# xinyiW915/ReLaX-VQA

Measured on AMD Instinct MI355X. Metric: clips/sec (32 sampled frames, 1080p) feature extraction, higher is better.
Workload: dtype f32 (fp32-grade split-operand arithmetic, fp32 accumulate: the whole ViT (GEMMs and attention), ResNet-50's stem, layer3 / layer4, and in layer1 / layer2 the 3x3 convolutions, every conv3 (back to back with its 3x3), the downsample convolutions and layer2's conv1 on fp32 operands as 2 fp16 planes x

## Files before the change

relax-vqa_amd/csrc/gemm_h2.hip:

```cpp
#include "relax_internal.h"
#include "host_logic.h"
#include "h2.h"
#include "gelu.h"

#ifndef H3_EP_FETCH_AHEAD
#define H3_EP_FETCH_AHEAD 0
#endif
#ifndef H2_STAMP
#define H2_STAMP(i_)
#define H2_STAMPS_BEFORE_LAUNCH(h_, p_, units_)
#define H2_STAMPS_AFTER_LAUNCH(h_, p_, units_, s_)
#endif
#ifndef H3_ABL_NO_A
#define H3_ABL_NO_A(taps_, perimg_, p_) false
#define H3_ABL_NO_OUT_H2(taps_, p_) false
#endif
#ifndef H3_KSTEP
#define H3_KSTEP(k_) (k_)
#endif

namespace relax {

typedef float h2k_f32x4 __attribute__((ext_vector_type(4)));
typedef float f32x4 __attribute__((ext_vector_type(4)));
// ... 90 lines not shown
    hipLaunchKernelGGL(to_h2_rows_kernel, dim3((unsigned)((rows + 3) / 4)), dim3(256), 0, s, x, ld, static_cast<char*>(y), K, rows, inv_scale);
    RELAX_HIP_CHECK(h, hipGetLastError());
    return RELAX_OK;
}

struct H2Params {
    const char* a;
    const char* w;
    const float* colscale;
    const float* rowscale;
    const float* bias;
    const float* residual;
    float* out;
    char* out_h2;
    float out_scale;
    float* partial;
    int M, N, K;
    int act;
    int no_split;
    int tiles_m, tiles_n, ntiles, group_m;
    int full_tiles, nsplit;
    int pixels, H, W, Cin, Ho, Wo, KW, stride, pad;
    int rows_per_img;
    const float* img_in_inv;
    const float* img_out_scale;
    unsigned* amax_out;
    const char* residual_h2;
    const float* img_res_inv;
    float* gap;
    int out_rows, gap_rows;
    unsigned long long* stamps;
};

__device__ inline int xcd_remap_h2(int b, int nwg) {
    const int q = nwg >> 3, r = nwg & 7, xcd = b & 7;
    const int base = xcd < r ? xcd * (q + 1) : r * (q + 1) + (xcd - r) * q;
    return base + (b >> 3);
}

#define H2_DMA(rsrc_, lds_off_, voff_, soff_)                                                                             \
    __builtin_amdgcn_raw_ptr_buffer_load_lds(rsrc_, (__attribute__((address_space(3))) void*)(smem + (lds_off_)), 16,     \
                                             voff_, soff_, 0, 0)
[[maybe_unused]] constexpr unsigned kH2OutOfRange = 0x80000000u;
constexpr int64_t kH2MaxRecords = 0x7ffffff0;

constexpr int H2_BM = 256, H2_BN = 256;
constexpr int H2_STAGE = (H2_BM + H2_BN) * kH2ChunkBytes;
constexpr int H2_PIECES = H2_STAGE / 1024;
[[maybe_unused]] constexpr int H2_PPW = H2_PIECES / 8;

template <int NSTG>
__global__ __launch_bounds__(512, 2) void gemm_h2(const H2Params p) {
#if __HIP_DEVICE_COMPILE__
    constexpr int BM = H2_BM, BN = H2_BN, STAGE = H2_STAGE, PPW = H2_PPW;
    extern __shared__ __attribute__((aligned(16))) char smem[];
    const int tid = threadIdx.x;
    const int lane = tid & 63;
    const int wave = __builtin_amdgcn_readfirstlane(tid >> 6);
    const int wm = wave >> 2, wn = wave & 3;

    int tile, kt_begin, kt_end, slice = -1, split_tile = 0;
    {
        const int nk_all = p.K >> 4;
        const int b = blockIdx.x;
        if (b < p.full_tiles) {
            tile = xcd_remap_h2(b, p.full_tiles);
            kt_begin = 0;
            kt_end = nk_all;
        } else {
            const int u = b - p.full_tiles;
            split_tile = u / p.nsplit;
            slice = u - split_tile * p.nsplit;
            tile = p.full_tiles + split_tile;
            kt_begin = (int)((int64_t)nk_all * slice / p.nsplit);
            kt_end = (int)((int64_t)nk_all * (slice + 1) / p.nsplit);
        }
    }
    int tm, tn;
    {
        const int per_group = p.group_m * p.tiles_n;
        const int g = tile / per_group;
        const int first = g * p.group_m;
        const int gsz = p.tiles_m - first < p.group_m ? p.tiles_m - first : p.group_m;
        const int w = tile - g * per_group;
        tm = first + w % gsz;
        tn = w / gsz;
    }
    const int m0 = tm * BM;
    const int n0 = tn * BN;
    H2_STAMP(0);

    const int64_t row_bytes = (int64_t)p.K * 4;
    __amdgpu_buffer_rsrc_t rsrc_a, rsrc_w;
    {
        const int64_t left = (int64_t)(p.M - m0) * row_bytes;
        rsrc_a = __builtin_amdgcn_make_buffer_rsrc(const_cast<char*>(p.a + (int64_t)m0 * row_bytes), 0,
                                                   (int)(left < kH2MaxRecords ? left : kH2MaxRecords), 0x00020000);
        rsrc_w = __builtin_amdgcn_make_buffer_rsrc(const_cast<char*>(p.w + (int64_t)n0 * row_bytes), 0, (int)(BN * row_bytes), 0x00020000);
    }
    unsigned voff_a, voff_w;
    {
        const int r = 32 * wave + (lane >> 1);
        voff_a = m0 + r < p.M ? (unsigned)(r * (int)row_bytes + (lane & 1) * 16) : kH2OutOfRange;
        voff_w = (unsigned)(r * (int)row_bytes + (lane & 1) * 16);
    }
    int d_kt = kt_begin;
#define H2_ISSUE_PIECE(st_, j_)                                                                                         \
    {                                                                                                                   \
        const int soff_ = d_kt * kH2ChunkBytes + ((j_) >> 1) * 32;                                                      \
        const int dst_ = (st_) * STAGE + ((j_) >> 1) * (STAGE / 2) + ((j_) & 1) * (BM * 32) + wave * 1024;               \
        if (((j_) & 1) == 0) { H2_DMA(rsrc_a, dst_, voff_a, soff_); }                                                    \
        else { H2_DMA(rsrc_w, dst_, voff_w, soff_); }                                                                    \
    }
#define H2_ISSUE(st_)                                                                                                   \
    {                                                                                                                   \
        _Pragma("unroll") for (int j = 0; j < PPW; ++j) H2_ISSUE_PIECE(st_, j);                                         \
        ++d_kt;                                                                                                         \
    }

    floatx4 acc[8][4];
#pragma unroll
    for (int i = 0; i < 8; ++i)
#pragma unroll
        for (int j = 0; j < 4; ++j)
#pragma unroll
            for (int r = 0; r < 4; ++r) acc[i][j][r] = 0.f;

    const int r16 = lane & 15, g16 = lane >> 4;
    const int a_hl = (g16 >> 1) * (STAGE / 2) + (wm * 128 + r16) * 32 + ((g16 & 1) << 4);
    const int b_hh = (BM + wn * 64 + r16) * 32 + ((g16 & 1) << 4);
    h2k_f16x8 xb[2][4][2], ya[2];
#define H2_READ_XB(set_, sp_)                                                                                           \
    _Pragma("unroll") for (int y = 0; y < 4; ++y) {                                                                     \
        xb[set_][y][0] = *reinterpret_cast<const h2k_f16x8*>((sp_) + b_hh + y * 16 * 32);                               \
        xb[set_][y][1] = *reinterpret_cast<const h2k_f16x8*>((sp_) + b_hh + y * 16 * 32 + STAGE / 2);                   \
    }
#define H2_READ_A(buf_, e_, sp_)                                                                                        \
    {                                                                                                                   \
        ya[buf_] = *reinterpret_cast<const h2k_f16x8*>((sp_) + a_hl + (e_) * 16 * 32);                                  \
        __builtin_amdgcn_sched_barrier(0);                        \
    }
#define H2_MFMAS(set_, buf_, e_)                                                                                        \
    {                                                                                                                   \
        _Pragma("unroll") for (int y = 0; y < 4; ++y)                                                                   \
            acc[e_][y] = __builtin_amdgcn_mfma_f32_16x16x32_f16(ya[buf_], xb[set_][y][1], acc[e_][y], 0, 0, 0);         \
        _Pragma("unroll") for (int y = 0; y < 4; ++y)                                                                   \
            acc[e_][y] = __builtin_amdgcn_mfma_f32_16x16x32_f16(ya[buf_], xb[set_][y][0], acc[e_][y], 0, 0, 0);         \
        __builtin_amdgcn_sched_barrier(0);        \
    }
#define H2_REGION(xs_, st_, has_next_, has_d_)                                                                          \
    {                                                                                                                   \
        const char* sn_ = smem + (((st_) + 1) % NSTG) * STAGE;                                                          \
        if (has_next_) {                                                                                                \
            if (has_d_) asm volatile("s_waitcnt vmcnt(%0) lgkmcnt(0)" ::"n"((NSTG - 2) * PPW) : "memory");              \
            else asm volatile("s_waitcnt vmcnt(0) lgkmcnt(0)" ::: "memory");                                            \
            __builtin_amdgcn_s_barrier();                                                                               \
            H2_READ_XB((xs_) ^ 1, sn_);                                                                                 \
            H2_READ_A(0, 0, sn_);                                                                                       \
        }                                                                                                               \
        H2_MFMAS(xs_, 1, 7);                                                                                            \
        if (has_next_) {                                                                                                \
            _Pragma("unroll") for (int e = 0; e < 7; ++e) {                                                             \
                H2_READ_A((e + 1) & 1, e + 1, sn_);                                                                     \
                if ((has_d_) && e < PPW) H2_ISSUE_PIECE(st_, e);                                                        \
                H2_MFMAS((xs_) ^ 1, e & 1, e);                                                                          \
            }                                                                                                           \
            if (has_d_) ++d_kt;                                                                                         \
        }                                                                                                               \
    }

    const int nk = kt_end - kt_begin;
    {
        const int pre = nk < NSTG ? nk : NSTG;
        for (int i = 0; i < pre; ++i) H2_ISSUE(i);
        if (pre >= 4) asm volatile("s_waitcnt vmcnt(%0)" ::"n"(3 * PPW) : "memory");
        else if (pre == 3) asm volatile("s_waitcnt vmcnt(%0)" ::"n"(2 * PPW) : "memory");
        else if (pre == 2) asm volatile("s_waitcnt vmcnt(%0)" ::"n"(PPW) : "memory");
        else asm volatile("s_waitcnt vmcnt(0)" ::: "memory");
    }
    __builtin_amdgcn_s_barrier();
    H2_READ_XB(0, smem);
    H2_READ_A(0, 0, smem);
    H2_STAMP(1);
#pragma unroll
    for (int e = 0; e < 7; ++e) {
        H2_READ_A((e + 1) & 1, e + 1, smem);
        H2_MFMAS(0, e & 1, e);
    }
    {
        constexpr int PERIOD = (NSTG % 2 == 0) ? NSTG : 2 * NSTG;
        int k = 0;
        for (; k + PERIOD + NSTG <= nk; k += PERIOD) {
#pragma unroll
            for (int i = 0; i < PERIOD; ++i) H2_REGION(i & 1, i % NSTG, true, true);
        }
        for (; k < nk; k += PERIOD) {
#pragma unroll
            for (int i = 0; i < PERIOD; ++i)
                if (k + i < nk) H2_REGION(i & 1, i % NSTG, k + i + 1 < nk, k + i + NSTG < nk);
        }
    }
#undef H2_REGION
#undef H2_MFMAS
#undef H2_READ_A
#undef H2_READ_XB
#undef H2_ISSUE
#undef H2_ISSUE_PIECE
    H2_STAMP(2);
    __syncthreads();

    float* stg = reinterpret_cast<float*>(smem);
    constexpr int LDC = BN + 4;
    constexpr int EP_ROWS = 64;
    constexpr int C8 = BN / 8;
    constexpr int NT = 512;
    static_assert(EP_ROWS * LDC * 4 <= NSTG * STAGE, "epilogue pass must fit the staging LDS");
    constexpr int EP_STEP = NT / C8;
    constexpr int EP_ITERS = EP_ROWS / EP_STEP;
    const bool planes = p.out_h2 != nullptr;
    const int lcA = planes ? (tid % C8) * 8 : (tid % C8) * 4;
    const int lcB = planes ? lcA + 4 : lcA + BN / 2;
    const int lr0 = tid / C8;
    const f32x4 zero4 = {0.f, 0.f, 0.f, 0.f};
    f32x4 bias_a = zero4, bias_b = zero4, cs_a = zero4, cs_b = zero4;
    if (slice < 0) {
        cs_a = *reinterpret_cast<const f32x4*>(p.colscale + n0 + lcA);
        cs_b = *reinterpret_cast<const f32x4*>(p.colscale + n0 + lcB);
        if (p.bias) {
            bias_a = *reinterpret_cast<const f32x4*>(p.bias + n0 + lcA);
            bias_b = *reinterpret_cast<const f32x4*>(p.bias + n0 + lcB);
        }
    }
    const bool interior = m0 + BM <= p.M;
#pragma unroll
    for (int pass = 0; pass < BM / EP_ROWS; ++pass) {
        if (pass > 0) __syncthreads();
        f32x4 ra[EP_ITERS], rb[EP_ITERS];
        float rs[EP_ITERS];
#pragma unroll
        for (int it = 0; it < EP_ITERS; ++it) {
            const int m = m0 + pass * EP_ROWS + it * EP_STEP + lr0;
            ra[it] = zero4;
            rb[it] = zero4;
            rs[it] = 1.f;
            if (slice < 0 && (interior || m < p.M)) {
                if (p.residual) {
                    const float* r = p.residual + (int64_t)m * p.N + n0;
                    ra[it] = *reinterpret_cast<const f32x4*>(r + lcA);
                    rb[it] = *reinterpret_cast<const f32x4*>(r + lcB);
                }
                if (p.rowscale) rs[it] = p.rowscale[m];
            }
        }
#pragma unroll
        for (int x = 0; x < 8; ++x) {
            const int rb0 = wm * 128 + x * 16;
            if (rb0 / EP_ROWS == pass) {
#pragma unroll
                for (int y = 0; y < 4; ++y)
#pragma unroll
                    for (int r = 0; r < 4; ++r) stg[(rb0 % EP_ROWS + 4 * g16 + r) * LDC + wn * 64 + y * 16 + r16] = acc[x][y][r];
            }
        }
        __syncthreads();
#pragma unroll
        for (int it = 0; it < EP_ITERS; ++it) {
            const int lr = it * EP_STEP + lr0;
            const int trow = pass * EP_ROWS + lr;
            const int m = m0 + trow;
            if (!interior && m >= p.M) continue;
            f32x4 va = *reinterpret_cast<const f32x4*>(stg + lr * LDC + lcA);
            f32x4 vb = *reinterpret_cast<const f32x4*>(stg + lr * LDC + lcB);
            if (slice >= 0) {
                float* o = p.partial + ((int64_t)split_tile * p.nsplit + slice) * (BM * BN) + (int64_t)trow * BN;
                *reinterpret_cast<f32x4*>(o + lcA) = va;
                *reinterpret_cast<f32x4*>(o + lcB) = vb;
                continue;
            }
            va = va * (cs_a * rs[it]) + bias_a;
            vb = vb * (cs_b * rs[it]) + bias_b;
            if (p.residual) {
                va += ra[it];
                vb += rb[it];
            }
            if (p.act == 1) {
                va = (f32x4){fmaxf(va.x, 0.f), fmaxf(va.y, 0.f), fmaxf(va.z, 0.f), fmaxf(va.w, 0.f)};
                vb = (f32x4){fmaxf(vb.x, 0.f), fmaxf(vb.y, 0.f), fmaxf(vb.z, 0.f), fmaxf(vb.w, 0.f)};
            } else if (p.act == 2) {
                va = gelu_erf4(va);
                vb = gelu_erf4(vb);
            }
            const int64_t o = (int64_t)m * p.N + n0;
            if (p.out) {
                *reinterpret_cast<f32x4*>(p.out + o + lcA) = va;
                *reinterpret_cast<f32x4*>(p.out + o + lcB) = vb;
            }
            if (p.out_h2) store_h2_x8(p.out_h2 + (int64_t)m * ((int64_t)p.N * 4), n0 + lcA, va, vb, p.out_scale);
        }
    }
    H2_STAMP(3);
#endif
}

constexpr int H3_STAGE = (H2_BM + H2_BN) * 128;
constexpr int H3_NSTG = 2;

__device__ inline float dpp_row_max(float v) {
#define H3_DPP_MAX(CTRL_) v = fmaxf(v, __builtin_bit_cast(float, __builtin_amdgcn_update_dpp(0, __builtin_bit_cast(int, v), CTRL_, 0xf, 0xf, true)))
    H3_DPP_MAX(0xB1);
    H3_DPP_MAX(0x4E);
    H3_DPP_MAX(0x141);
    H3_DPP_MAX(0x140);
#undef H3_DPP_MAX
    return v;
}

template <bool FOUR, bool TAPS = false, bool PERIMG = false>
__global__ __launch_bounds__(512, 2) void gemm_h3(const H2Params p) {
#if __HIP_DEVICE_COMPILE__
    constexpr int BM = H2_BM, BN = H2_BN, STAGE = H3_STAGE, NSTG = H3_NSTG, IMG = STAGE / 2;
    extern __shared__ __attribute__((aligned(16))) char smem[];
    const int tid = threadIdx.x;
    const int lane = tid & 63;
    const int wave = __builtin_amdgcn_readfirstlane(tid >> 6);
    const int wm = wave >> 2, wn = wave & 3;

    int tile, kt_begin, kt_end, slice = -1, split_tile = 0;
    {
        const int nk_all = p.K >> 5;
        const int b = blockIdx.x;
        if (b < p.full_tiles) {
            tile = xcd_remap_h2(b, p.full_tiles);
            kt_begin = 0;
            kt_end = nk_all;
        } else {
            const int u = b - p.full_tiles;
            split_tile = u / p.nsplit;
            slice = u - split_tile * p.nsplit;
            tile = p.full_tiles + split_tile;
            kt_begin = (int)((int64_t)nk_all * slice / p.nsplit);
            kt_end = (int)((int64_t)nk_all * (slice + 1) / p.nsplit);
        }
    }
    int tm, tn;
    {
        const int per_group = p.group_m * p.tiles_n;
        const int g = tile / per_group;
        const int first = g * p.group_m;
        const int gsz = p.tiles_m - first < p.group_m ? p.tiles_m - first : p.group_m;
        const int w = tile - g * per_group;
        tm = first + w % gsz;
        tn = w / gsz;
    }
    const int m0 = tm * BM;
    const int n0 = tn * BN;
#ifdef H3_STAGGER
    if (PERIMG && !TAPS && blockIdx.x < 256 && (blockIdx.x & 3)) {
        const unsigned long long t0 = __builtin_amdgcn_s_memtime(), wait = (unsigned long long)(blockIdx.x & 3) * (H3_STAGGER);
        while (__builtin_amdgcn_s_memtime() - t0 < wait) __builtin_amdgcn_s_sleep(32);
    }
#endif
    H2_STAMP(0);

    const int64_t row_bytes = (int64_t)p.K * 4;
    const int64_t arow_bytes = p.pixels ? (int64_t)p.Cin * 4 : row_bytes;
    const int img0 = p.pixels ? m0 / (p.Ho * p.Wo) : 0;
    __amdgpu_buffer_rsrc_t rsrc_a, rsrc_w;
    {
        const int64_t base = p.pixels ? (int64_t)img0 * p.H * p.W * arow_bytes : (int64_t)m0 * arow_bytes;
        const int64_t total = p.pixels ? (int64_t)(p.M / (p.Ho * p.Wo)) * p.H * p.W * arow_bytes : (int64_t)p.M * arow_bytes;
        const int64_t left = total - base;
        rsrc_a = __builtin_amdgcn_make_buffer_rsrc(const_cast<char*>(p.a + base), 0, (int)(left < kH2MaxRecords ? left : kH2MaxRecords), 0x00020000);
        rsrc_w = __builtin_amdgcn_make_buffer_rsrc(const_cast<char*>(p.w + (int64_t)n0 * row_bytes), 0, (int)(BN * row_bytes), 0x00020000);
    }
    unsigned voff[4];
    [[maybe_unused]] unsigned a_taps[2] = {0u, 0u};
    const int ntaps = TAPS ? p.K / p.Cin : 1;
#pragma unroll
    for (int q = 0; q < 4; ++q) {
        const int trow = (wave + 8 * q) * 16 + (lane >> 2);
        const int unit = (lane & 3) ^ ((4 - ((trow >> 2) & 3)) & 3);
        const int off = (unit >> 1) * kH2ChunkBytes + (unit & 1) * 16;
        if (q >= 2) {
            voff[q] = (unsigned)((trow - BM) * (int)row_bytes + off);
        } else if (m0 + trow >= p.M || H3_ABL_NO_A(TAPS, PERIMG, p)) {
            voff[q] = kH2OutOfRange;
        } else if (p.pixels) {
            const int m = m0 + trow;
            const int img = m / (p.Ho * p.Wo);
            const int rem = m - img * (p.Ho * p.Wo);
            const int oy = rem / p.Wo;
            const int ox = rem - oy * p.Wo;
            const int iy = oy * p.stride - p.pad, ix = ox * p.stride - p.pad;
            if (TAPS) {
                for (int t = 0, dy = 0, dx = 0; t < ntaps; ++t) {
                    if ((unsigned)(iy + dy) < (unsigned)p.H && (unsigned)(ix + dx) < (unsigned)p.W) a_taps[q] |= 1u << t;
                    if (++dx == p.KW) { dx = 0; ++dy; }
                }
            }
            voff[q] = (unsigned)((((img - img0) * p.H + iy) * p.W + ix) * (int)arow_bytes + off);
        } else {
            voff[q] = (unsigned)(trow * (int)arow_bytes + off);
        }
    }
    int d_kt = kt_begin;
    [[maybe_unused]] int d_cc = 0, d_tap = 0, d_dy = 0, d_dx = 0;
    [[maybe_unused]] const int cin_chunks = p.Cin >> 4;
    if (TAPS) {
        d_cc = kt_begin / ntaps;
        d_tap = kt_begin - d_cc * ntaps;
        d_dy = d_tap / p.KW;
        d_dx = d_tap - d_dy * p.KW;
    }
#define H3_ISSUE_PIECE(st_, j_)                                                                                         \
    {                                                                                                                   \
        const int dst_ = (st_) * STAGE + ((j_) >> 2) * IMG + (wave + 8 * ((j_) & 3)) * 1024;                             \
        if (((j_) & 3) < 2) {                                                                                           \
            if (TAPS) {                                                                                                 \
                const bool ok_ = (a_taps[(j_) & 1] >> d_tap) & 1u;                                                      \
                const int tapoff_ = (d_dy * p.W + d_dx) * (int)arow_bytes + d_cc * (2 * kH2ChunkBytes) + ((j_) >> 2) * 32; \
                H2_DMA(rsrc_a, dst_, ok_ ? voff[(j_) & 3] + (unsigned)tapoff_ : kH2OutOfRange, 0);                      \
            } else {                                                                                                    \
                H2_DMA(rsrc_a, dst_, voff[(j_) & 3], H3_KSTEP(d_kt) * (2 * kH2ChunkBytes) + ((j_) >> 2) * 32);          \
            }                                                                                                           \
        } else {                                                                                                        \
            const int wk_ = TAPS ? (d_tap * cin_chunks + 2 * d_cc) * kH2ChunkBytes : H3_KSTEP(d_kt) * (2 * kH2ChunkBytes); \
            H2_DMA(rsrc_w, dst_, voff[(j_) & 3], wk_ + ((j_) >> 2) * 32);                                                \
        }                                                                                                               \
    }
#define H3_ISSUE_ADVANCE()                                                                                              \
    {                                                                                                                   \
        ++d_kt;                                                                                                         \
        if (TAPS) {                                                                                                     \
            ++d_tap;                                                                                                    \
            ++d_dx;                                                                                                     \
            const bool wx_ = d_dx == p.KW;                                                                              \
            d_dx = wx_ ? 0 : d_dx;                                                                                      \
            d_dy += wx_ ? 1 : 0;                                                                                        \
            const bool wt_ = d_tap == ntaps;                                                                            \
            d_tap = wt_ ? 0 : d_tap;                                                                                    \
            d_dy = wt_ ? 0 : d_dy;                                                                                      \
            d_cc += wt_ ? 1 : 0;                                                                                        \
        }                                                                                                               \
    }

    floatx4 acc[8][4];
#pragma unroll
    for (int i = 0; i < 8; ++i)
#pragma unroll
        for (int j = 0; j < 4; ++j)
#pragma unroll
            for (int r = 0; r < 4; ++r) acc[i][j][r] = 0.f;

    const int r16 = lane & 15, g16 = lane >> 4;
    const int f16 = (4 - ((r16 >> 2) & 3)) & 3;
    const int a_h = (wm * 128 + r16) * 64 + ((g16 ^ f16) << 4);
    const int b_h = (BM + wn * 64 + r16) * 64 + ((g16 ^ f16) << 4);
    h2k_f16x8 xb[2][4][2], ya[2][2];
#define H3_READ_XB(set_, sp_)                                                                                           \
    _Pragma("unroll") for (int y = 0; y < 4; ++y) {                                                                     \
        xb[set_][y][0] = *reinterpret_cast<const h2k_f16x8*>((sp_) + b_h + y * 16 * 64);                                \
        xb[set_][y][1] = *reinterpret_cast<const h2k_f16x8*>((sp_) + b_h + y * 16 * 64 + IMG);                          \
    }
#define H3_READ_A(buf_, e_, sp_)                                                                                        \
    {                                                                                                                   \
        ya[buf_][0] = *reinterpret_cast<const h2k_f16x8*>((sp_) + a_h + (e_) * 16 * 64);                                \
        ya[buf_][1] = *reinterpret_cast<const h2k_f16x8*>((sp_) + a_h + (e_) * 16 * 64 + IMG);                          \
        __builtin_amdgcn_sched_barrier(0);                      \
    }
#define H3_MFMAS(set_, buf_, e_)                                                                                        \
    {                                                                                                                   \
        if (FOUR) {                                                                                                     \
            _Pragma("unroll") for (int y = 0; y < 4; ++y)                                                               \
                acc[e_][y] = __builtin_amdgcn_mfma_f32_16x16x32_f16(ya[buf_][1], xb[set_][y][1], acc[e_][y], 0, 0, 0);  \
        }                                                                                                               \
        _Pragma("unroll") for (int y = 0; y < 4; ++y)                                                                   \
            acc[e_][y] = __builtin_amdgcn_mfma_f32_16x16x32_f16(ya[buf_][1], xb[set_][y][0], acc[e_][y], 0, 0, 0);      \
        _Pragma("unroll") for (int y = 0; y < 4; ++y)                                                                   \
            acc[e_][y] = __builtin_amdgcn_mfma_f32_16x16x32_f16(ya[buf_][0], xb[set_][y][1], acc[e_][y], 0, 0, 0);      \
        _Pragma("unroll") for (int y = 0; y < 4; ++y)                                                                   \
            acc[e_][y] = __builtin_amdgcn_mfma_f32_16x16x32_f16(ya[buf_][0], xb[set_][y][0], acc[e_][y], 0, 0, 0);      \
        __builtin_amdgcn_sched_barrier(0);        \
    }
#define H3_ORDER(i_) (i_)
#define H3_REGION(xs_, has_next_, has_d_)                                                                               \
    {                                                                                                                   \
        const char* sn_ = smem + ((xs_) ^ 1) * STAGE;                                                                   \
        if (has_next_) {                                                                                                \
            asm volatile("s_waitcnt vmcnt(0) lgkmcnt(0)" ::: "memory");                                                 \
            __builtin_amdgcn_s_barrier();                                                                               \
            H3_READ_XB((xs_) ^ 1, sn_);                                                                                 \
            H3_READ_A(0, 0, sn_);                                                                                       \
            if (has_d_) H3_ISSUE_PIECE(xs_, H3_ORDER(0));                                                               \
        }                                                                                                               \
        H3_MFMAS(xs_, 1, 7);                                                                                            \
        if (has_next_) {                                                                                                \
            _Pragma("unroll") for (int e = 0; e < 7; ++e) {                                                             \
                H3_READ_A((e + 1) & 1, e + 1, sn_);                                                                     \
                if (has_d_) H3_ISSUE_PIECE(xs_, H3_ORDER(e + 1));                                                       \
                H3_MFMAS((xs_) ^ 1, e & 1, e);                                                                          \
            }                                                                                                           \
            if (has_d_) H3_ISSUE_ADVANCE();                                                                             \
        }                                                                                                               \
    }

    const int nk = kt_end - kt_begin;
    {
#pragma unroll
        for (int j = 0; j < 8; ++j) H3_ISSUE_PIECE(0, j);
        H3_ISSUE_ADVANCE();
        if (nk > 1) {
#pragma unroll
            for (int j = 0; j < 8; ++j) H3_ISSUE_PIECE(1, j);
            H3_ISSUE_ADVANCE();
            asm volatile("s_waitcnt vmcnt(8)" ::: "memory");
        } else {
            asm volatile("s_waitcnt vmcnt(0)" ::: "memory");
        }
    }
    __builtin_amdgcn_s_barrier();
    H3_READ_XB(0, smem);
    H3_READ_A(0, 0, smem);
    H2_STAMP(1);
#pragma unroll
    for (int e = 0; e < 7; ++e) {
        H3_READ_A((e + 1) & 1, e + 1, smem);
        H3_MFMAS(0, e & 1, e);
    }
    {
        int k = 0;
        for (; k + 3 < nk; k += 2) {
            H3_REGION(0, true, true);
            H3_REGION(1, true, true);
        }
        for (; k < nk; k += 2) {
            H3_REGION(0, k + 1 < nk, k + 2 < nk);
            if (k + 1 < nk) H3_REGION(1, k + 2 < nk, k + 3 < nk);
        }
    }
#undef H3_REGION
#undef H3_ORDER
#undef H3_MFMAS
#undef H3_READ_A
#undef H3_READ_XB
#undef H3_ISSUE_PIECE
#undef H3_ISSUE_ADVANCE
    H2_STAMP(2);
    __syncthreads();
    H2_STAMP(7);

    float* stg = reinterpret_cast<float*>(smem);
    constexpr int LDC = BN + 4;
    constexpr int EP_ROWS = 64;
    constexpr int C8 = BN / 8;
    constexpr int NT = 512;
    static_assert(EP_ROWS * LDC * 4 <= NSTG * STAGE, "epilogue pass must fit the staging LDS");
    constexpr int EP_STEP = NT / C8;
    constexpr int EP_ITERS = EP_ROWS / EP_STEP;
    const bool planes = p.out_h2 != nullptr || (PERIMG && p.residual_h2 != nullptr);
    const int lcA = planes ? (tid % C8) * 8 : (tid % C8) * 4;
    const int lcB = planes ? lcA + 4 : lcA + BN / 2;
    const int lr0 = tid / C8;
    const f32x4 zero4 = {0.f, 0.f, 0.f, 0.f};
    const f32x4 cs_a = *reinterpret_cast<const f32x4*>(p.colscale + n0 + lcA);
    const f32x4 cs_b = *reinterpret_cast<const f32x4*>(p.colscale + n0 + lcB);
    const __amdgpu_buffer_rsrc_t rs_bias = __builtin_amdgcn_make_buffer_rsrc(const_cast<float*>(p.bias), 0, p.bias ? p.N * 4 : 0, 0x00020000);
    const f32x4 bias_a = __builtin_bit_cast(f32x4, __builtin_amdgcn_raw_buffer_load_b128(rs_bias, (n0 + lcA) * 4, 0, 0));
    const f32x4 bias_b = __builtin_bit_cast(f32x4, __builtin_amdgcn_raw_buffer_load_b128(rs_bias, (n0 + lcB) * 4, 0, 0));
    const bool interior = m0 + BM <= p.M;
    unsigned* simg = reinterpret_cast<unsigned*>(smem + 96 * 1024);
    const int rpi = p.rows_per_img;
    const int img_first = rpi > 0 ? m0 / rpi : 0;
    const int row_first = m0 - img_first * rpi;
    const float rpi_inv = rpi > 0 ? 1.f / (float)rpi : 0.f;
    auto img_of_row = [&](int trow) -> int {
        const int x = row_first + trow;
        int q = (int)((float)x * rpi_inv);
        q -= (q * rpi > x) ? 1 : 0;
        q += ((q + 1) * rpi <= x) ? 1 : 0;
        return img_first + q;
    };
    const bool lds_amax = PERIMG && p.amax_out && slice < 0 && p.rows_per_img >= 18;
    if (lds_amax && tid < 16) simg[tid] = 0u;
    const int64_t tile_ofs = ((int64_t)m0 * p.N + n0) * 4;
    const unsigned row_pitch = (unsigned)p.N * 4u;
    const unsigned ofs_f = (unsigned)lr0 * row_pitch + (unsigned)lcA * 4u;
    const unsigned ofs_p = (unsigned)lr0 * row_pitch + (unsigned)h2_offset(lcA);
    const unsigned ofs_fb = (unsigned)(lcB - lcA) * 4u;
    const bool res_planes = PERIMG && p.residual_h2 != nullptr;
    const char* res_ptr = res_planes ? p.residual_h2 : reinterpret_cast<const char*>(p.residual);
    const int64_t res_left = (int64_t)p.M * p.N * 4 - tile_ofs;
    const __amdgpu_buffer_rsrc_t rs_res = __builtin_amdgcn_make_buffer_rsrc(
        const_cast<char*>(res_ptr) + (res_ptr ? tile_ofs : 0), 0, (res_ptr && slice < 0) ? (int)(res_left < kH2MaxRecords ? res_left : kH2MaxRecords) : 0, 0x00020000);
    const unsigned ofs_r = res_planes ? ofs_p : ofs_f, ofs_rb = res_planes ? 32u : ofs_fb;
    char* tile_out = reinterpret_cast<char*>(p.out) + tile_ofs;
    char* tile_out_h2 = p.out_h2 + tile_ofs;
    f32x4 ra[EP_ITERS], rb[EP_ITERS];
    float rs[EP_ITERS], os[EP_ITERS], rri[EP_ITERS];
    int im[EP_ITERS];
#define H3_EP_FETCH(P_, IT_)                                                                                                     \
    {                                                                                                                            \
        const int trow_ = (P_) * EP_ROWS + (IT_) * EP_STEP + lr0;                                                                \
        const int m_ = m0 + trow_;                                                                                               \
        const unsigned row_ofs_ = (unsigned)(((P_) * EP_ROWS + (IT_) * EP_STEP) * row_pitch);                                    \
        ra[IT_] = __builtin_bit_cast(f32x4, __builtin_amdgcn_raw_buffer_load_b128(rs_res, row_ofs_ + ofs_r, 0, 0));              \
        rb[IT_] = __builtin_bit_cast(f32x4, __builtin_amdgcn_raw_buffer_load_b128(rs_res, row_ofs_ + ofs_r + ofs_rb, 0, 0));     \
        rs[IT_] = 1.f;                                                                                                           \
        os[IT_] = p.out_scale;                                                                                                   \
        rri[IT_] = 1.f;                                                                                                          \
        im[IT_] = 0;                                                                                                             \
        if (slice < 0 && (interior || m_ < p.M)) {                                                                               \
            if (p.rowscale) rs[IT_] = p.rowscale[m_];                                                                            \
            if (PERIMG && rpi > 0) {                                                      \
                im[IT_] = img_of_row(trow_);                                                                                     \
                if (p.img_in_inv) rs[IT_] = p.img_in_inv[im[IT_]];                                                               \
                if (p.img_out_scale) os[IT_] = p.img_out_scale[im[IT_]];                                                         \
            }                                                                                                                    \
            if (res_planes) rri[IT_] = p.img_res_inv[im[IT_]];  \
        }                                                                                                                        \
    }
    constexpr bool EP_AHEAD = PERIMG && H3_EP_FETCH_AHEAD;
    if constexpr (EP_AHEAD) {
#pragma unroll
        for (int it = 0; it < EP_ITERS; ++it) H3_EP_FETCH(0, it);
    }
#pragma unroll
    for (int pass = 0; pass < BM / EP_ROWS; ++pass) {
        if (pass > 0) __syncthreads();
        if constexpr (!EP_AHEAD) {
#pragma unroll
            for (int it = 0; it < EP_ITERS; ++it) H3_EP_FETCH(pass, it);
        }
        if (pass == 0) H2_STAMP(4);
#pragma unroll
        for (int x = 0; x < 8; ++x) {
            const int rb0 = wm * 128 + x * 16;
            if (rb0 / EP_ROWS == pass) {
#pragma unroll
                for (int y = 0; y < 4; ++y)
#pragma unroll
                    for (int r = 0; r < 4; ++r) stg[(rb0 % EP_ROWS + 4 * g16 + r) * LDC + wn * 64 + y * 16 + r16] = acc[x][y][r];
            }
        }
        __syncthreads();
        if (pass == 0) H2_STAMP(5);
        if constexpr (!EP_AHEAD) {
#pragma unroll
            for (int it = 0; it < EP_ITERS; ++it) {
                asm volatile("" : "+v"(ra[it]), "+v"(rb[it]), "+v"(rs[it]));
                if constexpr (PERIMG) asm volatile("" : "+v"(os[it]), "+v"(rri[it]));
            }
        }
#pragma unroll
        for (int it = 0; it < EP_ITERS; ++it) {
            const int lr = it * EP_STEP + lr0;
            const int trow = pass * EP_ROWS + lr;
            const int m = m0 + trow;
            f32x4 xa = ra[it], xb = rb[it];
            const float rs_it = rs[it], os_it = os[it];
            const int im_it = im[it];
            if (res_planes) {
                const h2_u32x4 hi = __builtin_bit_cast(h2_u32x4, xa), lo = __builtin_bit_cast(h2_u32x4, xb);
                const float ri = rri[it];
#define H2_LO16(u_) ((float)__builtin_bit_cast(_Float16, (unsigned short)((u_) & 0xffffu)))
#define H2_HI16(u_) ((float)__builtin_bit_cast(_Float16, (unsigned short)((u_) >> 16)))
                xa = (f32x4){H2_LO16(hi.x) + H2_LO16(lo.x), H2_HI16(hi.x) + H2_HI16(lo.x), H2_LO16(hi.y) + H2_LO16(lo.y),
                             H2_HI16(hi.y) + H2_HI16(lo.y)} * ri;
                xb = (f32x4){H2_LO16(hi.z) + H2_LO16(lo.z), H2_HI16(hi.z) + H2_HI16(lo.z), H2_LO16(hi.w) + H2_LO16(lo.w),
                             H2_HI16(hi.w) + H2_HI16(lo.w)} * ri;
#undef H2_LO16
#undef H2_HI16
            }
            if constexpr (EP_AHEAD) {
                if (pass + 1 < BM / EP_ROWS) H3_EP_FETCH(pass + 1, it);
            }
            if (!interior && m >= p.M) continue;
            f32x4 va = *reinterpret_cast<const f32x4*>(stg + lr * LDC + lcA);
            f32x4 vb = *reinterpret_cast<const f32x4*>(stg + lr * LDC + lcB);
            if (slice >= 0) {
                float* o = p.partial + ((int64_t)split_tile * p.nsplit + slice) * (BM * BN) + (int64_t)trow * BN;
                *reinterpret_cast<f32x4*>(o + lcA) = va;
                *reinterpret_cast<f32x4*>(o + lcB) = vb;
                continue;
            }
            va = va * (cs_a * rs_it) + bias_a;
            vb = vb * (cs_b * rs_it) + bias_b;
            if (res_ptr) {
                va += xa;
                vb += xb;
            }
            if (p.act == 1) {
                va = (f32x4){fmaxf(va.x, 0.f), fmaxf(va.y, 0.f), fmaxf(va.z, 0.f), fmaxf(va.w, 0.f)};
                vb = (f32x4){fmaxf(vb.x, 0.f), fmaxf(vb.y, 0.f), fmaxf(vb.z, 0.f), fmaxf(vb.w, 0.f)};
            } else if (p.act == 2) {
                va = gelu_erf4(va);
                vb = gelu_erf4(vb);
            }
            const unsigned row_ofs = (unsigned)((pass * EP_ROWS + it * EP_STEP) * row_pitch);
            if (p.out && (!PERIMG || m < p.out_rows)) {
                char* o = tile_out + (size_t)(unsigned)(row_ofs + ofs_f);
                *reinterpret_cast<f32x4*>(o) = va;
                *reinterpret_cast<f32x4*>(o + ofs_fb) = vb;
            }
            if (PERIMG && p.gap) {
                *reinterpret_cast<f32x4*>(stg + lr * LDC + lcA) = va;
                *reinterpret_cast<f32x4*>(stg + lr * LDC + lcB) = vb;
            }
            if (p.out_h2 && !H3_ABL_NO_OUT_H2(TAPS, p)) {
                h2_u32x4 hi, lo;
                split2_x8(va * os_it, vb * os_it, hi, lo);
                char* o = tile_out_h2 + (size_t)(unsigned)(row_ofs + ofs_p);
                *reinterpret_cast<h2_u32x4*>(o) = hi;
                *reinterpret_cast<h2_u32x4*>(o + 32) = lo;
            }
            if (PERIMG && p.amax_out) {
                float mx = fmaxf(fmaxf(fmaxf(va.x, va.y), fmaxf(va.z, va.w)), fmaxf(fmaxf(vb.x, vb.y), fmaxf(vb.z, vb.w)));
                mx = dpp_row_max(mx);
                if ((tid & 15) == 0) {
                    if (lds_amax) atomicMax(simg + (im_it - img_first), __float_as_uint(mx));
                    else atomicMax(p.amax_out + im_it, __float_as_uint(mx));
                }
            }
        }
        if (pass == 0) H2_STAMP(6);
        if (PERIMG && p.gap && slice < 0) {
            __syncthreads();
            for (int e = tid; e < (EP_ROWS / 4) * BN; e += NT) {
                const int g = e / BN, col = e - g * BN;
                const int mg = m0 + pass * EP_ROWS + g * 4;
                if (mg < p.gap_rows) {
                    float t = 0.f;
#pragma unroll
                    for (int r = 0; r < 4; ++r) t += stg[(g * 4 + r) * LDC + col];
                    p.gap[(int64_t)(mg >> 2) * p.N + n0 + col] = t;
                }
            }
        }
    }
#undef H3_EP_FETCH
    if (lds_amax) {
        __syncthreads();
        if (tid < 16 && simg[tid] != 0u) atomicMax(p.amax_out + img_first + tid, simg[tid]);
    }
    H2_STAMP(3);
#endif
}

__global__ __launch_bounds__(256) void splitk_finish_h2(const H2Params p) {
    constexpr int BM = H2_BM, BN = H2_BN;
    const int split_tile = blockIdx.y;
    const int tile = p.full_tiles + split_tile;
    int tm, tn;
    {
        const int per_group = p.group_m * p.tiles_n;
        const int g = tile / per_group;
        const int first = g * p.group_m;
        const int gsz = p.tiles_m - first < p.group_m ? p.tiles_m - first : p.group_m;
        const int w = tile - g * per_group;
        tm = first + w % gsz;
        tn = w / gsz;
    }
    const int m0 = tm * BM;
    const int n0 = tn * BN;
    const int e8 = blockIdx.x * 256 + threadIdx.x;
    const int lr = e8 / (BN / 8), lc = (e8 % (BN / 8)) * 8;
    const int m = m0 + lr;
    __shared__ unsigned s_mx[8];
    const int img_b0 = p.rows_per_img > 0 ? (m0 + blockIdx.x * 8) / p.rows_per_img : 0;
    if (threadIdx.x < 8) s_mx[threadIdx.x] = 0u;
    __syncthreads();
    if (m < p.M) {
    const float* pt = p.partial + (int64_t)split_tile * p.nsplit * (BM * BN) + lr * BN + lc;
    f32x4 va = *reinterpret_cast<const f32x4*>(pt), vb = *reinterpret_cast<const f32x4*>(pt + 4);
    for (int k = 1; k < p.nsplit; ++k) {
        va += *reinterpret_cast<const f32x4*>(pt + (int64_t)k * (BM * BN));
        vb += *reinterpret_cast<const f32x4*>(pt + (int64_t)k * (BM * BN) + 4);
    }
    const int64_t o = (int64_t)m * p.N + n0 + lc;
    float rs = p.rowscale ? p.rowscale[m] : 1.f, os = p.out_scale;
    const int img = p.rows_per_img > 0 ? m / p.rows_per_img : 0;
    if (p.rows_per_img > 0) {
        if (p.img_in_inv) rs = p.img_in_inv[img];
        if (p.img_out_scale) os = p.img_out_scale[img];
    }
    va = va * (*reinterpret_cast<const f32x4*>(p.colscale + n0 + lc) * rs);
    vb = vb * (*reinterpret_cast<const f32x4*>(p.colscale + n0 + lc + 4) * rs);
    if (p.bias) {
        va += *reinterpret_cast<const f32x4*>(p.bias + n0 + lc);
        vb += *reinterpret_cast<const f32x4*>(p.bias + n0 + lc + 4);
    }
    if (p.residual) {
        va += *reinterpret_cast<const f32x4*>(p.residual + o);
        vb += *reinterpret_cast<const f32x4*>(p.residual + o + 4);
    }
    if (p.act == 1) {
        va = (f32x4){fmaxf(va.x, 0.f), fmaxf(va.y, 0.f), fmaxf(va.z, 0.f), fmaxf(va.w, 0.f)};
        vb = (f32x4){fmaxf(vb.x, 0.f), fmaxf(vb.y, 0.f), fmaxf(vb.z, 0.f), fmaxf(vb.w, 0.f)};
    } else if (p.act == 2) {
        va = gelu_erf4(va);
        vb = gelu_erf4(vb);
    }
    if (p.out && m < p.out_rows) {
        *reinterpret_cast<f32x4*>(p.out + o) = va;
        *reinterpret_cast<f32x4*>(p.out + o + 4) = vb;
    }
    if (p.out_h2) store_h2_x8(p.out_h2 + (int64_t)m * ((int64_t)p.N * 4), n0 + lc, va, vb, os);
    if (p.amax_out) {
        float mx = fmaxf(fmaxf(fmaxf(va.x, va.y), fmaxf(va.z, va.w)), fmaxf(fmaxf(vb.x, vb.y), fmaxf(vb.z, vb.w)));
#pragma unroll
        for (int o = 16; o >= 1; o >>= 1) mx = fmaxf(mx, __shfl_xor(mx, o));
        if ((threadIdx.x & 31) == 0) atomicMax(&s_mx[(img - img_b0) & 7], __float_as_uint(mx));
    }
    }
    if (p.amax_out) {
        __syncthreads();
        if (threadIdx.x < 8 && s_mx[threadIdx.x] != 0u) atomicMax(p.amax_out + img_b0 + threadIdx.x, s_mx[threadIdx.x]);
    }
}

template <int FORM>
static int launch_h2_variant(relax_handle* h, H2Params& p, hipStream_t s) {
    constexpr int BM = H2_BM, BN = H2_BN;
    constexpr bool BK32 = FORM >= 2;
    const bool can_split = h->gemm.split_k && !p.no_split && !p.gap && !p.residual_h2;
    RELAX_TRY(plan_tiles(h, p, BM, BN, 256, BK32 ? p.K / 32 : p.K / 16, BK32 ? 4 : 8, can_split));
    constexpr size_t lds = BK32 ? (size_t)H3_NSTG * H3_STAGE : (size_t)(FORM == 1 ? 4 : 3) * H2_STAGE;
    auto kernel = [] {
        if constexpr (FORM == 0) return &gemm_h2<3>;
        else if constexpr (FORM == 1) return &gemm_h2<4>;
        else if constexpr (FORM == 2) return &gemm_h3<false>;
        else if constexpr (FORM == 3) return &gemm_h3<true>;
        else if constexpr (FORM == 4) return &gemm_h3<false, true, true>;
        else return &gemm_h3<false, false, true>;
    }();
    static std::atomic<bool> lds_allowed[kMaxDevices];
    RELAX_TRY(allow_dynamic_lds(h, {reinterpret_cast<const void*>(kernel)}, lds, lds_allowed));
    const int units = p.full_tiles + (p.ntiles - p.full_tiles) * p.nsplit;
    H2_STAMPS_BEFORE_LAUNCH(h, p, units);
    hipLaunchKernelGGL(kernel, dim3(units), dim3(512), lds, s, p);
    H2_STAMPS_AFTER_LAUNCH(h, p, units, s);
    if (p.nsplit > 1)
        hipLaunchKernelGGL(splitk_finish_h2, dim3(BM * BN / 8 / 256, p.ntiles - p.full_tiles), dim3(256), 0, s, p);
    RELAX_HIP_CHECK(h, hipGetLastError());
    return RELAX_OK;
}

int launch_gemm_h2(relax_handle* h, const GemmDescH2& d, hipStream_t s) {
    H2Params p{};
    p.a = static_cast<const char*>(d.a);
    p.w = static_cast<const char*>(d.w);
    p.colscale = d.colscale; p.rowscale = d.rowscale;
    p.bias = d.bias; p.residual = d.residual; p.out = d.out; p.out_h2 = static_cast<char*>(d.out_h2); p.out_scale = d.out_scale;
    p.M = d.M; p.N = d.N; p.K = d.K; p.act = d.act; p.no_split = d.no_split;
    const bool conv = d.pixels != 0;
    const bool taps = conv && d.KH * d.KW > 1;
    if (conv) {
        p.pixels = 1; p.H = d.H; p.W = d.W; p.Cin = d.Cin; p.Ho = d.Ho; p.Wo = d.Wo; p.KW = d.KW; p.stride = d.stride; p.pad = d.pad;
        RELAX_REQUIRE(h, d.Nimg > 0 && d.M == d.Nimg * d.Ho * d.Wo && d.K == d.KH * d.KW * d.Cin && d.Cin % 32 == 0 && d.KH * d.KW <= 32 &&
                             (taps || d.pad == 0) && d.stride >= 1 && (int64_t)d.H * d.W * d.Cin * 4 * 4 < kH2MaxRecords,
                      "f16x2 conv: bad geometry (Cin=%d must be a multiple of 32, at most 32 taps, M = Nimg*Ho*Wo, K = KH*KW*Cin)", d.Cin);
    }
    p.rows_per_img = d.rows_per_img; p.img_in_inv = d.img_in_inv; p.img_out_scale = d.img_out_scale; p.amax_out = d.amax_out;
    p.residual_h2 = static_cast<const char*>(d.residual_h2); p.img_res_inv = d.img_res_inv; p.gap = d.gap_groups;
    p.out_rows = d.out_rows > 0 && d.out_rows < d.M ? d.out_rows : d.M;
    p.gap_rows = d.gap_rows > 0 && d.gap_rows < d.M ? d.gap_rows : d.M;
    RELAX_REQUIRE(h, !(d.residual && d.residual_h2) && (!d.residual_h2 || (d.img_res_inv && d.rows_per_img > 0)), "f16x2 gemm: bad residual");
    RELAX_REQUIRE(h, !d.gap_groups || (d.rows_per_img > 0 && d.rows_per_img % 4 == 0), "f16x2 conv: the fused spatial mean needs Ho*Wo %% 4 == 0");
    RELAX_REQUIRE(h, d.rows_per_img > 0 || (!d.img_in_inv && !d.img_out_scale && !d.amax_out), "f16x2 gemm: per-image tables need rows_per_img");
    RELAX_REQUIRE(h, conv || (d.rows_per_img == 0 && !d.residual_h2 && !d.gap_groups && d.out_rows == 0),
                  "f16x2 gemm: per-image scales, plane residuals, fused means and out_rows belong to the convolution form");
    RELAX_REQUIRE(h, p.M > 0 && p.N > 0 && p.K > 0, "f16x2 gemm: empty problem M=%d N=%d K=%d", p.M, p.N, p.K);
    RELAX_REQUIRE(h, p.K % 16 == 0 && p.N % 256 == 0, "f16x2 gemm: K=%d must be a multiple of 16 and N=%d of 256", p.K, p.N);
    RELAX_REQUIRE(h, (int64_t)p.K * 4 * 256 < kH2MaxRecords, "f16x2 gemm: K=%d too large", p.K);
    RELAX_REQUIRE(h, d.a && d.w && d.colscale && (d.out || d.out_h2 || d.gap_groups), "f16x2 gemm: missing operand / no output requested");
    RELAX_REQUIRE(h, !d.amax_out || d.act == 1, "f16x2 gemm: amax_out needs act == 1 (ReLU): the bit-ordered maximum is valid for non-negative outputs only");
    RELAX_REQUIRE(h, !d.out_h2 || d.img_out_scale || (d.out_scale > 0.f && d.out_scale < 3.0e38f), "f16x2 gemm: the plane output needs its scale");
    auto aligned16 = [](const void* q) { return (reinterpret_cast<uintptr_t>(q) & 15) == 0; };
    RELAX_REQUIRE(h, aligned16(d.a) && aligned16(d.w) && aligned16(d.colscale) && aligned16(d.bias) && aligned16(d.residual) && aligned16(d.out) &&
                         aligned16(d.out_h2),
                  "f16x2 gemm: every operand pointer must be 16-byte aligned");
    const double flops = 2.0 * p.M * (double)p.N * (double)p.K;
    const double bytes = 4.0 * ((conv ? (double)d.Nimg * d.H * d.W * d.Cin : (double)p.M * p.K) + (double)p.N * p.K) +
                         (double)p.M * p.N * ((d.out ? 4.0 : 0.0) + (d.out_h2 ? 4.0 : 0.0) + (d.residual ? 4.0 : 0.0));
    int span;
    RELAX_TRY(prof_begin(h, s, conv ? 5 : 6, flops, &span, bytes));
    int rc;
    if (conv) {
        RELAX_REQUIRE(h, p.K % 32 == 0, "f16x2 conv: K=%d must be a multiple of 32", p.K);
        rc = taps ? launch_h2_variant<4>(h, p, s) : launch_h2_variant<5>(h, p, s);
    } else if (h->gemm.h2_form == 0 || p.K % 32 != 0) rc = h->gemm.h2_stages == 4 ? launch_h2_variant<1>(h, p, s) : launch_h2_variant<0>(h, p, s);
    else if (h->gemm.h2_form == 2 || p.K < 256) rc = launch_h2_variant<3>(h, p, s);
    else rc = launch_h2_variant<2>(h, p, s);
    if (rc != RELAX_OK) { prof_abort(h, span); return rc; }
    RELAX_TRY(prof_end(h, s, span));
    return RELAX_OK;
}

}
```

Baseline: 118.0.

## Split gemm_h3 staging into separate A and W rings with a deeper A ring

Splits the single combined A+W LDS stage ring of the h3 GEMM into independent operand rings, so A and W can use different pipeline depths. The plain form (FORM 2/3) now uses three A stages and two W stages, with loads issued further ahead and a partial vmcnt wait instead of draining all loads before each barrier. This targets global-load latency that stays exposed with only double buffering. In exchange it uses more LDS per block, which may lower occupancy under launch_bounds(512,2), and it adds period-6 unrolling and more complex issue scheduling.

```diff
diff --git a/relax-vqa_amd/csrc/gemm_h2.hip b/relax-vqa_amd/csrc/gemm_h2.hip
--- a/relax-vqa_amd/csrc/gemm_h2.hip
+++ b/relax-vqa_amd/csrc/gemm_h2.hip
@@ -416,8 +416,24 @@
 #endif
 }
 
-constexpr int H3_STAGE = (H2_BM + H2_BN) * 128;
-constexpr int H3_NSTG = 2;
+constexpr int H3_OPSTAGE = H2_BM * 128;
+static_assert(H2_BM == H2_BN, "gemm_h3: the operand rings share their stage size");
+#ifndef H3_PLAIN_STAGES
+#define H3_PLAIN_STAGES 3, 2, 0
+#endif
+#ifndef H3_CONV1_STAGES
+#define H3_CONV1_STAGES 2, 2, 0
+#endif
+#ifndef H3_TAPS_STAGES
+#define H3_TAPS_STAGES 2, 2, 0
+#endif
+struct H3Rings { int a, b, order; };
+constexpr H3Rings h3_rings(bool taps, bool perimg) { return taps ? H3Rings{H3_TAPS_STAGES} : perimg ? H3Rings{H3_CONV1_STAGES} : H3Rings{H3_PLAIN_STAGES}; }
+constexpr size_t h3_lds_bytes(bool taps, bool perimg) { return (size_t)(h3_rings(taps, perimg).a + h3_rings(taps, perimg).b) * H3_OPSTAGE; }
+#ifndef H2_STAMP_LATCH
+#define H2_STAMP_LATCH(v_)
+#define H2_STAMP_PUT(i_, v_)
+#endif
 
 __device__ inline float dpp_row_max(float v) {
 #define H3_DPP_MAX(CTRL_) v = fmaxf(v, __builtin_bit_cast(float, __builtin_amdgcn_update_dpp(0, __builtin_bit_cast(int, v), CTRL_, 0xf, 0xf, true)))
@@ -429,10 +445,13 @@
     return v;
 }
 
-template <bool FOUR, bool TAPS = false, bool PERIMG = false>
-__global__ __launch_bounds__(512, 2) void gemm_h3(const H2Params p) {
 #if __HIP_DEVICE_COMPILE__
-    constexpr int BM = H2_BM, BN = H2_BN, STAGE = H3_STAGE, NSTG = H3_NSTG, IMG = STAGE / 2;
+template <bool FOUR, bool TAPS, bool PERIMG, int ASTG, int BSTG, int ORDER>
+__device__ __forceinline__ void gemm_h3_body(const H2Params& p) {
+    constexpr int BM = H2_BM, BN = H2_BN, OPSTG = H3_OPSTAGE, IMG = OPSTG / 2, B0 = ASTG * OPSTG;
+    constexpr int LA = ASTG - 2, LB = BSTG - 2;
+    static_assert(LA >= 0 && LB >= 0 && LA + LB <= 1 && (ORDER == 0 || ORDER == 1), "gemm_h3: 2 + 2, 3 + 2 or 2 + 3 stages");
+    constexpr int WAITN = ORDER == 0 ? 4 : 2;
     extern __shared__ __attribute__((aligned(16))) char smem[];
     const int tid = threadIdx.x;
     const int lane = tid & 63;
@@ -517,45 +536,80 @@
             voff[q] = (unsigned)(trow * (int)arow_bytes + off);
         }
     }
-    int d_kt = kt_begin;
-    [[maybe_unused]] int d_cc = 0, d_tap = 0, d_dy = 0, d_dx = 0;
+    int dA_kt = kt_begin;
+    [[maybe_unused]] int dA_cc = 0, dA_tap = 0, dA_dy = 0, dA_dx = 0;
     [[maybe_unused]] const int cin_chunks = p.Cin >> 4;
     if (TAPS) {
-        d_cc = kt_begin / ntaps;
-        d_tap = kt_begin - d_cc * ntaps;
-        d_dy = d_tap / p.KW;
-        d_dx = d_tap - d_dy * p.KW;
-    }
-#define H3_ISSUE_PIECE(st_, j_)                                                                                         \
-    {                                                                                                                   \
-        const int dst_ = (st_) * STAGE + ((j_) >> 2) * IMG + (wave + 8 * ((j_) & 3)) * 1024;                             \
-        if (((j_) & 3) < 2) {                                                                                           \
-            if (TAPS) {                                                                                                 \
-                const bool ok_ = (a_taps[(j_) & 1] >> d_tap) & 1u;                                                      \
-                const int tapoff_ = (d_dy * p.W + d_dx) * (int)arow_bytes + d_cc * (2 * kH2ChunkBytes) + ((j_) >> 2) * 32; \
-                H2_DMA(rsrc_a, dst_, ok_ ? voff[(j_) & 3] + (unsigned)tapoff_ : kH2OutOfRange, 0);                      \
-            } else {                                                                                                    \
-                H2_DMA(rsrc_a, dst_, voff[(j_) & 3], H3_KSTEP(d_kt) * (2 * kH2ChunkBytes) + ((j_) >> 2) * 32);          \
-            }                                                                                                           \
+        dA_cc = kt_begin / ntaps;
+        dA_tap = kt_begin - dA_cc * ntaps;
+        dA_dy = dA_tap / p.KW;
+        dA_dx = dA_tap - dA_dy * p.KW;
+    }
+    [[maybe_unused]] int dW_kt_own = dA_kt, dW_cc_own = dA_cc, dW_tap_own = dA_tap;
+    int &dW_kt = LA + LB > 0 ? dW_kt_own : dA_kt, &dW_cc = LA + LB > 0 ? dW_cc_own : dA_cc, &dW_tap = LA + LB > 0 ? dW_tap_own : dA_tap;
+#define H3_ISSUE_A(st_, i_)                                                                                             \
+    {                                                                                                                   \
+        const int dst_ = (st_) * OPSTG + ((i_) >> 1) * IMG + (wave + 8 * ((i_) & 1)) * 1024;                             \
+        if (TAPS) {                                                                                                     \
+            const bool ok_ = (a_taps[(i_) & 1] >> dA_tap) & 1u;                                                         \
+            const int tapoff_ = (dA_dy * p.W + dA_dx) * (int)arow_bytes + dA_cc * (2 * kH2ChunkBytes) + ((i_) >> 1) * 32; \
+            H2_DMA(rsrc_a, dst_, ok_ ? voff[(i_) & 1] + (unsigned)tapoff_ : kH2OutOfRange, 0);                          \
         } else {                                                                                                        \
-            const int wk_ = TAPS ? (d_tap * cin_chunks + 2 * d_cc) * kH2ChunkBytes : H3_KSTEP(d_kt) * (2 * kH2ChunkBytes); \
-            H2_DMA(rsrc_w, dst_, voff[(j_) & 3], wk_ + ((j_) >> 2) * 32);                                                \
+            H2_DMA(rsrc_a, dst_, voff[(i_) & 1], H3_KSTEP(dA_kt) * (2 * kH2ChunkBytes) + ((i_) >> 1) * 32);             \
         }                                                                                                               \
     }
-#define H3_ISSUE_ADVANCE()                                                                                              \
-    {                                                                                                                   \
-        ++d_kt;                                                                                                         \
+#define H3_ISSUE_W(st_, i_)                                                                                             \
+    {                                                                                                                   \
+        const int dst_ = B0 + (st_) * OPSTG + ((i_) >> 1) * IMG + (wave + 8 * ((i_) & 1)) * 1024;                        \
+        const int wk_ = TAPS ? (dW_tap * cin_chunks + 2 * dW_cc) * kH2ChunkBytes : H3_KSTEP(dW_kt) * (2 * kH2ChunkBytes); \
+        H2_DMA(rsrc_w, dst_, voff[2 + ((i_) & 1)], wk_ + ((i_) >> 1) * 32);                                              \
+    }
+#define H3_ADVANCE_A()                                                                                                  \
+    {                                                                                                                   \
+        ++dA_kt;                                                                                                        \
         if (TAPS) {                                                                                                     \
-            ++d_tap;                                                                                                    \
-            ++d_dx;                                                                                                     \
-            const bool wx_ = d_dx == p.KW;                                                                              \
-            d_dx = wx_ ? 0 : d_dx;                                                                                      \
-            d_dy += wx_ ? 1 : 0;                                                                                        \
-            const bool wt_ = d_tap == ntaps;                                                                            \
-            d_tap = wt_ ? 0 : d_tap;                                                                                    \
-            d_dy = wt_ ? 0 : d_dy;                                                                                      \
-            d_cc += wt_ ? 1 : 0;                                                                                        \
+            ++dA_tap;                                                                                                   \
+            ++dA_dx;                                                                                                    \
+            const bool wx_ = dA_dx == p.KW;                                                                             \
+            dA_dx = wx_ ? 0 : dA_dx;                                                                                    \
+            dA_dy += wx_ ? 1 : 0;                                                                                       \
+            const bool wt_ = dA_tap == ntaps;                                                                           \
+            dA_tap = wt_ ? 0 : dA_tap;                                                                                  \
+            dA_dy = wt_ ? 0 : dA_dy;                                                                                    \
+            dA_cc += wt_ ? 1 : 0;                                                                                       \
         }                                                                                                               \
+    }
+#define H3_ADVANCE_W()                                                                                                  \
+    if (LA + LB > 0) {                                                                                                  \
+        ++dW_kt;                                                                                                        \
+        if (TAPS) {                                                                                                     \
+            ++dW_tap;                                                                                                   \
+            const bool wt_ = dW_tap == ntaps;                                                                           \
+            dW_tap = wt_ ? 0 : dW_tap;                                                                                  \
+            dW_cc += wt_ ? 1 : 0;                                                                                       \
+        }                                                                                                               \
+    }
+#define H3_ISSUE_SLOT(sa_, sb_, s_, has_a_, has_b_)                                                                     \
+    {                                                                                                                   \
+        const bool grouped_ = LA + LB > 0 && ORDER == 0;                                                                \
+        const bool second_ = grouped_ ? (s_) >= 4 : ((s_) & 3) >= 2;                \
+        const bool is_a_ = LA + LB == 0 ? !second_ : second_ == (LA == 1);      \
+        const int i_ = grouped_ ? (s_) & 3 : ((s_) >> 2) * 2 + ((s_) & 1);                                              \
+        if (is_a_) {                                                                                                    \
+            if (has_a_) H3_ISSUE_A(sa_, i_);                                                                            \
+        } else {                                                                                                        \
+            if (has_b_) H3_ISSUE_W(sb_, i_);                                                                            \
+        }                                                                                                               \
+    }
+#define H3_ISSUE_STEP_A(step_)                                                                                          \
+    {                                                                                                                   \
+        _Pragma("unroll") for (int i = 0; i < 4; ++i) H3_ISSUE_A((step_) % ASTG, i);                                    \
+        H3_ADVANCE_A();                                                                                                 \
+    }
+#define H3_ISSUE_STEP_W(step_)                                                                                          \
+    {                                                                                                                   \
+        _Pragma("unroll") for (int i = 0; i < 4; ++i) H3_ISSUE_W((step_) % BSTG, i);                                    \
+        H3_ADVANCE_W();                                                                                                 \
     }
 
     floatx4 acc[8][4];
@@ -569,7 +623,7 @@
     const int r16 = lane & 15, g16 = lane >> 4;
     const int f16 = (4 - ((r16 >> 2) & 3)) & 3;
     const int a_h = (wm * 128 + r16) * 64 + ((g16 ^ f16) << 4);
-    const int b_h = (BM + wn * 64 + r16) * 64 + ((g16 ^ f16) << 4);
+    const int b_h = (wn * 64 + r16) * 64 + ((g16 ^ f16) << 4);
     h2k_f16x8 xb[2][4][2], ya[2][2];
 #define H3_READ_XB(set_, sp_)                                                                                           \
     _Pragma("unroll") for (int y = 0; y < 4; ++y) {                                                                     \
@@ -596,69 +650,106 @@
             acc[e_][y] = __builtin_amdgcn_mfma_f32_16x16x32_f16(ya[buf_][0], xb[set_][y][0], acc[e_][y], 0, 0, 0);      \
         __builtin_amdgcn_sched_barrier(0);        \
     }
-#define H3_ORDER(i_) (i_)
-#define H3_REGION(xs_, has_next_, has_d_)                                                                               \
-    {                                                                                                                   \
-        const char* sn_ = smem + ((xs_) ^ 1) * STAGE;                                                                   \
+#define H3_REGION(k6_, has_next_, has_e_, has_l_)                                                                       \
+    {                                                                                                                   \
+        const char* sa_ = smem + (((k6_) + 1) % ASTG) * OPSTG;                                                          \
+        const char* sb_ = smem + B0 + (((k6_) + 1) % BSTG) * OPSTG;                                                     \
+        const bool has_a_ = LA ? (has_l_) : (has_e_), has_b_ = LB ? (has_l_) : (has_e_);                                \
         if (has_next_) {                                                                                                \
-            asm volatile("s_waitcnt vmcnt(0) lgkmcnt(0)" ::: "memory");                                                 \
+            if (LA + LB > 0 && (has_e_)) asm volatile("s_waitcnt vmcnt(%0) lgkmcnt(0)" ::"n"(WAITN) : "memory");        \
+            else asm volatile("s_waitcnt vmcnt(0) lgkmcnt(0)" ::: "memory");                                            \
             __builtin_amdgcn_s_barrier();                                                                               \
-            H3_READ_XB((xs_) ^ 1, sn_);                                                                                 \
-            H3_READ_A(0, 0, sn_);                                                                                       \
-            if (has_d_) H3_ISSUE_PIECE(xs_, H3_ORDER(0));                                                               \
+            H3_READ_XB(((k6_) + 1) & 1, sb_);                                                                           \
+            H3_READ_A(0, 0, sa_);                                                                                       \
+            H3_ISSUE_SLOT(((k6_) + 2 + LA) % ASTG, ((k6_) + 2 + LB) % BSTG, 0, has_a_, has_b_);                         \
         }                                                                                                               \
-        H3_MFMAS(xs_, 1, 7);                                                                                            \
+        H3_MFMAS((k6_) & 1, 1, 7);                                                                                      \
         if (has_next_) {                                                                                                \
             _Pragma("unroll") for (int e = 0; e < 7; ++e) {                                                             \
-                H3_READ_A((e + 1) & 1, e + 1, sn_);                                                                     \
-                if (has_d_) H3_ISSUE_PIECE(xs_, H3_ORDER(e + 1));                                                       \
-                H3_MFMAS((xs_) ^ 1, e & 1, e);                                                                          \
+                H3_READ_A((e + 1) & 1, e + 1, sa_);                                                                     \
+                H3_ISSUE_SLOT(((k6_) + 2 + LA) % ASTG, ((k6_) + 2 + LB) % BSTG, e + 1, has_a_, has_b_);                 \
+                H3_MFMAS(((k6_) + 1) & 1, e & 1, e);                                                                    \
             }                                                                                                           \
-            if (has_d_) H3_ISSUE_ADVANCE();                                                                             \
+            if (has_a_) H3_ADVANCE_A();                                                                                 \
+            if (has_b_) H3_ADVANCE_W();                                                                                 \
         }                                                                                                               \
     }
 
     const int nk = kt_end - kt_begin;
-    {
-#pragma unroll
-        for (int j = 0; j < 8; ++j) H3_ISSUE_PIECE(0, j);
-        H3_ISSUE_ADVANCE();
+    if (LA + LB == 0) {
+#pragma unroll
+        for (int j = 0; j < 8; ++j) H3_ISSUE_SLOT(0, 0, j, true, true);
+        H3_ADVANCE_A();
+        H3_ADVANCE_W();
         if (nk > 1) {
 #pragma unroll
-            for (int j = 0; j < 8; ++j) H3_ISSUE_PIECE(1, j);
-            H3_ISSUE_ADVANCE();
+            for (int j = 0; j < 8; ++j) H3_ISSUE_SLOT(1, 1, j, true, true);
+            H3_ADVANCE_A();
+            H3_ADVANCE_W();
             asm volatile("s_waitcnt vmcnt(8)" ::: "memory");
         } else {
             asm volatile("s_waitcnt vmcnt(0)" ::: "memory");
         }
+    } else {
+        if (LA) {
+            H3_ISSUE_STEP_W(0);
+            H3_ISSUE_STEP_A(0);
+        } else {
+            H3_ISSUE_STEP_A(0);
+            H3_ISSUE_STEP_W(0);
+        }
+        if (nk > 1) {
+            if (LA) {
+                H3_ISSUE_STEP_W(1);
+                H3_ISSUE_STEP_A(1);
+            } else {
+                H3_ISSUE_STEP_A(1);
+                H3_ISSUE_STEP_W(1);
+            }
+        }
+        if (nk > 2) {
+            if (LA) H3_ISSUE_STEP_A(2) else H3_ISSUE_STEP_W(2)
+            asm volatile("s_waitcnt vmcnt(12)" ::: "memory");
+        } else if (nk > 1) {
+            asm volatile("s_waitcnt vmcnt(8)" ::: "memory");
+        } else {
+            asm volatile("s_waitcnt vmcnt(0)" ::: "memory");
+        }
     }
     __builtin_amdgcn_s_barrier();
-    H3_READ_XB(0, smem);
+    H3_READ_XB(0, smem + B0);
     H3_READ_A(0, 0, smem);
-    H2_STAMP(1);
+    H2_STAMP_LATCH(stamp1);
 #pragma unroll
     for (int e = 0; e < 7; ++e) {
         H3_READ_A((e + 1) & 1, e + 1, smem);
         H3_MFMAS(0, e & 1, e);
     }
     {
+        constexpr int PERIOD = LA + LB > 0 ? 6 : 2;
         int k = 0;
-        for (; k + 3 < nk; k += 2) {
-            H3_REGION(0, true, true);
-            H3_REGION(1, true, true);
-        }
-        for (; k < nk; k += 2) {
-            H3_REGION(0, k + 1 < nk, k + 2 < nk);
-            if (k + 1 < nk) H3_REGION(1, k + 2 < nk, k + 3 < nk);
+        for (; k + PERIOD + 1 + LA + LB < nk; k += PERIOD) {
+#pragma unroll
+            for (int i = 0; i < PERIOD; ++i) H3_REGION(i, true, true, true);
+        }
+        for (; k < nk; k += PERIOD) {
+#pragma unroll
+            for (int i = 0; i < PERIOD; ++i)
+                if (k + i < nk) H3_REGION(i, k + i + 1 < nk, k + i + 2 < nk, k + i + 3 < nk);
         }
     }
 #undef H3_REGION
-#undef H3_ORDER
+#undef H3_ISSUE_STEP_W
+#undef H3_ISSUE_STEP_A
+#undef H3_ISSUE_SLOT
+#undef H3_ADVANCE_W
+#undef H3_ADVANCE_A
+#undef H3_ISSUE_W
+#undef H3_ISSUE_A
 #undef H3_MFMAS
 #undef H3_READ_A
 #undef H3_READ_XB
-#undef H3_ISSUE_PIECE
-#undef H3_ISSUE_ADVANCE
+    H2_STAMP_PUT(1, stamp1);
     H2_STAMP(2);
     __syncthreads();
     H2_STAMP(7);
@@ -668,7 +759,7 @@
     constexpr int EP_ROWS = 64;
     constexpr int C8 = BN / 8;
     constexpr int NT = 512;
-    static_assert(EP_ROWS * LDC * 4 <= NSTG * STAGE, "epilogue pass must fit the staging LDS");
+    static_assert(EP_ROWS * LDC * 4 <= 96 * 1024 && 96 * 1024 + 64 <= (ASTG + BSTG) * OPSTG, "epilogue pass must fit the staging LDS");
     constexpr int EP_STEP = NT / C8;
     constexpr int EP_ITERS = EP_ROWS / EP_STEP;
     const bool planes = p.out_h2 != nullptr || (PERIMG && p.residual_h2 != nullptr);
@@ -857,6 +948,14 @@
         if (tid < 16 && simg[tid] != 0u) atomicMax(p.amax_out + img_first + tid, simg[tid]);
     }
     H2_STAMP(3);
+}
+#endif
+
+template <bool FOUR, bool TAPS = false, bool PERIMG = false>
+__global__ __launch_bounds__(512, 2) void gemm_h3(const H2Params p) {
+#if __HIP_DEVICE_COMPILE__
+    constexpr H3Rings R = h3_rings(TAPS, PERIMG);
+    gemm_h3_body<FOUR, TAPS, PERIMG, R.a, R.b, R.order>(p);
 #endif
 }
 
@@ -938,7 +1037,7 @@
     constexpr bool BK32 = FORM >= 2;
     const bool can_split = h->gemm.split_k && !p.no_split && !p.gap && !p.residual_h2;
     RELAX_TRY(plan_tiles(h, p, BM, BN, 256, BK32 ? p.K / 32 : p.K / 16, BK32 ? 4 : 8, can_split));
-    constexpr size_t lds = BK32 ? (size_t)H3_NSTG * H3_STAGE : (size_t)(FORM == 1 ? 4 : 3) * H2_STAGE;
+    constexpr size_t lds = BK32 ? h3_lds_bytes(FORM == 4, FORM >= 4) : (size_t)(FORM == 1 ? 4 : 3) * H2_STAGE;
     auto kernel = [] {
         if constexpr (FORM == 0) return &gemm_h2<3>;
         else if constexpr (FORM == 1) return &gemm_h2<4>;
```

New measurement: 120.4, median of 6. +2.0%, better.
